# Jamie725/Multimodal-Object-Detection-via-Probabilistic-Ensembling

Measured on AMD Instinct MI355X. Metric: RGB+T frame-pairs/sec (FLIR-aligned 640x512, two R101-FPN detectors + ProbEn), higher is better.
Workload: dtype f16; 1 GPU; configs[2]: FLIR RGB + thermal two-detector ProbEn (probEn/v-avg), batch 32 per GPU, R101-FPN x2, 640x512 -> 800x1000 (padded 800x1024), K=3, random-init weights; batch_per_gpu=32, input_residency=frames resident in HBM before the timed region (no H2D inside it), schedule=two detector streams, staggered by res3, batches back to back

## Files before the change

### include/proben_hip.h

```cpp
#ifndef PROBEN_HIP_H
#define PROBEN_HIP_H

#include <stddef.h>
#include <stdint.h>

#ifdef __cplusplus
extern "C" {
#endif

#define PE_OK 0
#define PE_ERR_INVALID_ARG (-1)
#define PE_ERR_UNSUPPORTED (-2)
#define PE_ERR_HIP (-3)

#define PE_SCORE_PROBEN 0
#define PE_SCORE_AVG 1
#define PE_SCORE_MAX 2
#define PE_SCORE_PROBEN_BINARY 3
#define PE_SCORE_PROBEN_LOGP 4
#define PE_BOX_VAVG 0
#define PE_BOX_SAVG 1
#define PE_BOX_AVG 2
#define PE_BOX_ARGMAX 3

// ... 168 lines not shown
                             int32_t src_c, int32_t ch0, int32_t nch, int32_t flip_rgb, int32_t dst_h, int32_t dst_w,
                             int32_t pad_h, int32_t pad_w, const float* mean_host, const float* std_host, void* dst,
                             void* stream);
int pe_preprocess_pack_pil_u8(const void* src, int32_t num_images, int32_t src_h, int32_t src_w, int32_t src_c,
                              int32_t ch0, int32_t nch, int32_t flip_rgb, int32_t dst_h, int32_t dst_w, int32_t pad_h,
                              int32_t pad_w, const float* mean_host, const float* std_host, const int32_t* xtab,
                              int32_t xk, const int32_t* ytab, int32_t yk, void* dst, void* stream);
int pe_fusion_input_pack(const void* thermal, const void* rgb, int32_t num_images, int32_t th_h, int32_t th_w, int32_t rgb_h,
                         int32_t rgb_w, int32_t ch0, int32_t nch, int32_t dst_h, int32_t dst_w, int32_t pad_h, int32_t pad_w,
                         int32_t pad_multiple, const float* mean_host, const float* std_host, void* dst, void* stream);
int pe_maxpool3x3s2_nhwc(const void* in, void* out, int32_t N, int32_t H, int32_t W, int32_t C, void* stream);
int pe_subsample2_nhwc(const void* in, void* out, int32_t N, int32_t H, int32_t W, int32_t C, void* stream);
int pe_stem_conv7x7_maxpool_f16(const void* x, const void* w_packed, const float* bias, void* out, int32_t N,
                                int32_t H, int32_t W, void* stream);

#define PE_NMS_TRICK 0
#define PE_NMS_CLASS 1
size_t pe_nms_scratch_bytes(int32_t B, int32_t n_max);
int pe_nms_batched(const float* boxes, const float* scores, const int32_t* idxs, const int32_t* counts,
                   const uint8_t* valid, int32_t B, int32_t n_max, float iou_thresh, int32_t mode,
                   int32_t max_out, int32_t* out_keep, int32_t* out_counts, void* scratch,
                   size_t scratch_bytes, void* stream);

int pe_rpn_select_topk(const float* const* level_heads_host, const int32_t* level_hw_host,
                       const int32_t* level_stride_host, const float* cell_anchors_host,
                       int32_t num_levels, int32_t N, int32_t head_stride, int32_t pre_nms_topk,
                       const int32_t* image_hw, float scale_clamp, float* cand_boxes, float* cand_scores,
                       int32_t* cand_level, uint8_t* cand_valid, int32_t cand_per_image, void* scratch,
                       size_t scratch_bytes, void* stream);
size_t pe_rpn_scratch_bytes(const int32_t* level_hw_host, int32_t num_levels, int32_t N);
int pe_gather_boxes(const float* boxes, const float* scores, const int32_t* keep, const int32_t* counts,
                    int32_t N, int32_t n_in, int32_t max_out, float* out_boxes, float* out_scores,
                    void* stream);

int pe_box2box_apply_deltas(const float* deltas, const float* boxes, int32_t N, int32_t k, const float* weights_host,
                            float scale_clamp, float* out, void* stream);
int pe_grid_anchors(const float* cell_anchors, int32_t num_cell_anchors, int32_t H, int32_t W, int32_t stride,
                    float offset, float* out, void* stream);

int pe_sgd_momentum_f32(float* params, const float* grads, float* momentum_buf, void* fp16_shadow, int64_t n, float lr,
                        float momentum, float weight_decay, float grad_scale, int32_t first_step, void* stream);

int pe_roi_align_nhwc(const void* const* feats_host, const int32_t* feat_hw_host, const float* scales_host,
                      int32_t num_levels, int32_t N, int32_t C, int32_t dtype, const float* rois,
                      int32_t rois_have_batch_index, int32_t num_rois, int32_t per_image,
                      const int32_t* counts, int32_t pooled_h, int32_t pooled_w, int32_t sampling_ratio,
                      int32_t aligned, void* output, int32_t* out_level, void* stream);

int pe_roi_align_nhwc_sorted(const void* const* feats_host, const int32_t* feat_hw_host, const float* scales_host,
                             int32_t num_levels, int32_t N, int32_t C, int32_t dtype, const float* boxes, int32_t per_image,
                             const int32_t* counts, int32_t pooled_h, int32_t pooled_w, int32_t sampling_ratio,
                             int32_t aligned, void* output, int32_t* out_level, int32_t* order_workspace, void* stream);

int pe_roi_align_backward_nhwc(const void* grad_output, int32_t dtype, const int32_t* feat_hw_host, const float* scales_host,
                               int32_t num_levels, int32_t N, int32_t C, const float* rois, int32_t rois_have_batch_index,
                               int32_t num_rois, int32_t per_image, const int32_t* counts, int32_t pooled_h,
                               int32_t pooled_w, int32_t sampling_ratio, int32_t aligned, float* const* grad_feats_host,
                               void* stream);

int pe_boxhead_candidates(const float* head, int32_t head_stride, int32_t N, int32_t per_image,
                          int32_t num_classes, const int32_t* prop_counts, const float* proposals,
                          const int32_t* image_hw, const float* reg_weights_host, float scale_clamp,
                          float score_thresh, int32_t cand_max, float* cand_boxes, float* cand_scores,
                          int32_t* cand_class, int32_t* cand_rows, int32_t* cand_counts, int32_t* cand_total,
                          float* probs, void* stream);
int pe_boxhead_finalize(const float* head, int32_t head_stride, int32_t N, int32_t per_image,
// ... 19 lines not shown
```

### multimodal-object-detection-via-probabilistic-ensembling_amd/_lib.py

```python
import ctypes
import os

import torch

_PKG = os.path.dirname(os.path.abspath(__file__))
LIB_PATH = os.path.join(_PKG, "libproben_hip.so")
_lib = None

c_void_p, c_int, c_double, c_float = ctypes.c_void_p, ctypes.c_int32, ctypes.c_double, ctypes.c_float
c_size_t = ctypes.c_size_t

SIGNATURES = {
    "pe_version": [],
    "pe_proben_pack_detections": [c_void_p] * 6 + [c_int] * 6 + [c_void_p] * 9,
    "pe_proben_pack_logits": [c_void_p] * 6 + [c_int] * 6 + [c_void_p] * 9,
    "pe_proben_pack_log_posteriors": [c_void_p] * 6 + [c_int] * 6 + [c_void_p] * 10,
    "pe_log_softmax": [c_void_p, ctypes.c_int64, c_int, c_double, c_void_p, c_void_p],
    "pe_proben_fuse_batch_logp": [c_void_p] * 8 + [c_int] * 4 + [c_double] * 3 + [c_void_p] * 6 + [c_void_p],
    "pe_calibrated_softmax": [c_void_p, ctypes.c_int64, c_int, c_double, c_void_p, c_void_p],
    "pe_temperature_nll": [c_void_p, c_void_p, ctypes.c_int64, c_int, c_void_p, c_int, c_void_p, c_void_p, c_void_p, c_void_p],
    "pe_match_ground_truth": [c_void_p] * 6 + [c_int, c_double, c_int] + [c_void_p] * 4,
    "pe_variance_stats": [c_void_p] * 4 + [ctypes.c_int64, ctypes.c_int64, c_void_p, c_double] + [c_void_p] * 4,
    "pe_proben_pack_calibrated": [c_void_p] * 9 + [c_int] * 6 + [c_void_p] * 10,
    "pe_proben_fuse_batch_pooled": [c_void_p] * 9 + [c_int] * 4 + [c_double] * 3 + [c_void_p] * 2 + [c_int] + [c_void_p] * 6 + [c_void_p],
    "pe_proben_fuse_batch_posterior": [c_void_p] * 9 + [c_int] * 4 + [c_double] * 3 + [c_void_p] * 2 + [c_int] + [c_void_p] * 9 + [c_void_p],
    "pe_proben_fuse_batch_presence": [c_void_p] * 9 + [c_int] * 4 + [c_double] * 3 + [c_void_p] * 3 + [c_int] + [c_void_p] * 10 + [c_void_p],
    "pe_bias_nll": [c_void_p, c_void_p, c_int, c_int, c_void_p, c_int, c_void_p, c_void_p, c_void_p, c_void_p],
    "pe_proben_pack_pooled": [c_void_p] * 9 + [c_int] * 6 + [c_void_p] * 11,
    "pe_pool_nll": [c_void_p, c_void_p, ctypes.c_int64, c_int, c_void_p, ctypes.c_int64, c_void_p, c_void_p, c_int, c_void_p, c_void_p,
                    c_int, c_int, c_void_p, c_void_p, c_void_p, c_void_p],
    "pe_reliability_logits": [c_void_p] * 3 + [ctypes.c_int64, c_int, c_double, c_int] + [c_void_p] * 5,
    "pe_reliability_scores": [c_void_p] * 2 + [ctypes.c_int64, c_int] + [c_void_p] * 5,
    "pe_proben_fuse_batch": [c_void_p] * 8 + [c_int] * 5 + [c_double] * 3 + [c_void_p] * 5 + [c_void_p],
    "pe_conv2d_nhwc_f16": [c_void_p] * 5 + [c_int] * 14 + [c_void_p],
    "pe_conv_wd_supported": [c_int] * 6,
    "pe_conv_wd_pack_weights": [c_void_p] * 2 + [c_int] * 3 + [c_void_p],
    "pe_conv3x3_wd_f16": [c_void_p] * 4 + [c_int] * 7 + [c_void_p],
    "pe_conv_wd_pack_tail": [c_void_p] * 2 + [c_int] * 2 + [c_void_p],
    "pe_bottleneck_tail_wd_f16": [c_void_p] * 7 + [c_int] * 5 + [c_void_p],
    "pe_bneck64_packed_bytes": [c_int] * 2,
    "pe_bneck64_pack": [c_void_p] * 6,
    "pe_bneck64_f16": [c_void_p] * 9 + [c_int] * 5 + [c_void_p],
    "pe_conv_wd_pack_head": [c_void_p] * 2 + [c_int] * 2 + [c_void_p],
    "pe_conv3x3_wd_rpn_head_f16": [c_void_p] * 6 + [c_int] * 4 + [c_void_p],
    "pe_preprocess_pack": [c_void_p] + [c_int] * 11 + [c_void_p] * 4,
    "pe_preprocess_pack_batch": [c_void_p] + [c_int] * 12 + [c_void_p] * 4,
    "pe_preprocess_pack_pil_u8": [c_void_p] + [c_int] * 11 + [c_void_p] * 2 + [c_void_p, c_int, c_void_p, c_int] + [c_void_p] * 2,
    "pe_fusion_input_pack": [c_void_p] * 2 + [c_int] * 12 + [c_void_p] * 4,
    "pe_maxpool3x3s2_nhwc": [c_void_p] * 2 + [c_int] * 4 + [c_void_p],
    "pe_subsample2_nhwc": [c_void_p] * 2 + [c_int] * 4 + [c_void_p],
    "pe_stem_conv7x7_maxpool_f16": [c_void_p] * 4 + [c_int] * 3 + [c_void_p],
    "pe_nms_scratch_bytes": [c_int, c_int],
    "pe_nms_batched": [c_void_p] * 5 + [c_int, c_int, c_float, c_int, c_int] + [c_void_p] * 3 + [c_size_t, c_void_p],
    "pe_rpn_select_topk": [c_void_p] * 4 + [c_int] * 4 + [c_void_p, c_float] + [c_void_p] * 4 + [c_int, c_void_p, c_size_t, c_void_p],
    "pe_rpn_scratch_bytes": [c_void_p, c_int, c_int],
    "pe_box2box_apply_deltas": [c_void_p] * 2 + [c_int] * 2 + [c_void_p, c_float, c_void_p, c_void_p],
    "pe_grid_anchors": [c_void_p, c_int, c_int, c_int, c_int, c_float, c_void_p, c_void_p],
    "pe_gather_boxes": [c_void_p] * 4 + [c_int] * 3 + [c_void_p] * 3,
    "pe_roi_align_nhwc": [c_void_p] * 3 + [c_int] * 4 + [c_void_p] + [c_int] * 3 + [c_void_p] + [c_int] * 4 + [c_void_p] * 3,
    "pe_roi_align_nhwc_sorted": [c_void_p] * 3 + [c_int] * 4 + [c_void_p] + [c_int] + [c_void_p] + [c_int] * 4 + [c_void_p] * 4,
    "pe_sgd_momentum_f32": [c_void_p] * 4 + [ctypes.c_int64] + [ctypes.c_float] * 4 + [c_int, c_void_p],
    "pe_roi_align_backward_nhwc": [c_void_p, c_int, c_void_p, c_void_p, c_int, c_int, c_int, c_void_p, c_int, c_int, c_int, c_void_p, c_int, c_int, c_int, c_int, c_void_p, c_void_p],
    "pe_boxhead_candidates": [c_void_p, c_int, c_int, c_int, c_int] + [c_void_p] * 4 + [c_float, c_float, c_int] + [c_void_p] * 8,
    "pe_cocoeval_bbox": [c_void_p] * 6 + [ctypes.c_int64] + [c_void_p] * 4 + [ctypes.c_int64, c_int, c_int, c_void_p, c_int,
                         c_void_p, c_int, c_void_p, c_int, c_void_p, c_int, c_int, c_void_p, c_void_p],
    "pe_boxhead_finalize": [c_void_p] + [c_int] * 7 + [c_void_p] * 18,
}
_RESTYPE = {"pe_last_error": ctypes.c_char_p, "pe_nms_scratch_bytes": ctypes.c_size_t, "pe_rpn_scratch_bytes": ctypes.c_size_t,
             "pe_bneck64_packed_bytes": ctypes.c_size_t}


TEST_HOOKS = {"pe_test_set_conv_policy": [c_int, c_int], "pe_test_set_wd9_mode": [c_int], "pe_test_wd9_takes": [c_int] * 5, "pe_test_wd9_head_takes": [c_int] * 3, "pe_test_set_wd9_wgs": [c_int, c_int], "pe_test_set_ring_wgs": [c_int], "pe_test_set_roi_fast": [c_int], "pe_test_set_nms_presorted": [c_int]}


class HipLibraryError(RuntimeError):
    pass


def lib():
    global _lib
    if _lib is None:
        if not os.path.exists(LIB_PATH):
            raise HipLibraryError(
                f"{LIB_PATH} is missing: run `python -c 'import __graft_entry__ as g; g.build()'` "
                "(hipcc --offload-arch=gfx950).  proben_amd has no CPU fallback.")
        L = ctypes.CDLL(LIB_PATH)
        L.pe_last_error.restype = ctypes.c_char_p
        L.pe_last_error.argtypes = []
        for name, args in SIGNATURES.items():
            fn = getattr(L, name)
            fn.argtypes = args
            fn.restype = _RESTYPE.get(name, ctypes.c_int)
        _lib = L
    return _lib


LAB_HOOKS = {"pe_test_set_ring_ablation": [c_int]}


def test_hooks():
    L = lib()
# ... 31 lines not shown
```

### multimodal-object-detection-via-probabilistic-ensembling_amd/csrc/nms.hip

```cpp
#include "common.h"
#include "test_hooks.h"

namespace {

constexpr int kSortThreads = 1024;
__device__ int g_presorted_path = 1;

__device__ __forceinline__ unsigned ordered_desc(float s) {
    s += 0.0f;
    unsigned u = __float_as_uint(s);
    u ^= (u >> 31) ? 0xFFFFFFFFu : 0x80000000u;
    return ~u;
}

struct NmsArgs {
    const float* boxes;
    const float* scores;
    const int32_t* idxs;
    const int32_t* counts;
    const uint8_t* valid;
    int B, n_max, n_pad;
    float thr;
    int mode, max_out;
    float* sboxes;
    int32_t* sidx;
    int32_t* scls;
    int32_t* nvalid;
    unsigned* sord;
    int32_t* seg_start;
    int32_t* nseg;
    unsigned long long* mask;
    int words;
    int32_t* out_keep;
// ... 123 lines not shown
__global__ __launch_bounds__(64) void nms_mask_kernel(NmsArgs a) {
    const int b = blockIdx.z;
    const int nv = a.nvalid[b];
    const int row0 = blockIdx.y * 64, col0 = blockIdx.x * 64;
    if (row0 >= nv || col0 >= nv || col0 + 63 < row0) return;
    __shared__ float cb[64][4];
    __shared__ int cc[64];
    const int t = threadIdx.x;
    const float* sb = a.sboxes + (size_t)b * a.n_max * 4;
    {
        const int* cls = a.scls + (size_t)b * a.n_max;
        const unsigned row_last = (unsigned)cls[min(row0 + 63, nv - 1)] & 0x3FFFFu, col_first = (unsigned)cls[col0] & 0x3FFFFu;
        if (col_first > row_last) {
            if (row0 + t < nv) a.mask[((size_t)b * a.n_max + row0 + t) * a.words + blockIdx.x] = 0ull;
            return;
        }
    }
    if (col0 + t < nv) {
        cb[t][0] = sb[(col0 + t) * 4]; cb[t][1] = sb[(col0 + t) * 4 + 1];
        cb[t][2] = sb[(col0 + t) * 4 + 2]; cb[t][3] = sb[(col0 + t) * 4 + 3];
        cc[t] = a.scls[(size_t)b * a.n_max + col0 + t];
    }
    __syncthreads();
    const int r = row0 + t;
    if (r >= nv) return;
    const float x1 = sb[r * 4], y1 = sb[r * 4 + 1], x2 = sb[r * 4 + 2], y2 = sb[r * 4 + 3];
    const float ar = (x2 - x1) * (y2 - y1);
    const int rc = a.scls[(size_t)b * a.n_max + r];
    unsigned long long bits = 0;
    const int jn = min(64, nv - col0);
    for (int j = (col0 == row0 ? t + 1 : 0); j < jn; ++j) {
        if (col0 + j <= r) continue;
        if (cc[j] != rc) continue;
        const float w = fmaxf(0.f, fminf(x2, cb[j][2]) - fmaxf(x1, cb[j][0]));
        const float h = fmaxf(0.f, fminf(y2, cb[j][3]) - fmaxf(y1, cb[j][1]));
        const float inter = w * h;
        const float aj = (cb[j][2] - cb[j][0]) * (cb[j][3] - cb[j][1]);
        const float iou = inter / (ar + aj - inter);
        if (iou > a.thr) bits |= 1ull << j;
    }
    a.mask[((size_t)b * a.n_max + r) * a.words + blockIdx.x] = bits;
}

constexpr int kScanThreads = 1024;
constexpr int kMergeSegs = 16;
__global__ __launch_bounds__(kScanThreads) void nms_scan_order_kernel(NmsArgs a) {
    extern __shared__ __attribute__((aligned(16))) unsigned char smem[];
    unsigned short* kept_pos = reinterpret_cast<unsigned short*>(smem);
    unsigned* flags = reinterpret_cast<unsigned*>(smem + (((size_t)a.n_max * 2 + 15) & ~(size_t)15));
    __shared__ int total_s;
    __shared__ int seg_p0_s[kMergeSegs], seg_kept_s[kMergeSegs];
    const int b = blockIdx.x, tid = threadIdx.x, lane = tid & 63, wave = tid >> 6;
    const int nv = a.nvalid[b];
    const int nseg = a.nseg[b];
    const unsigned long long* mk = a.mask + (size_t)b * a.n_max * a.words;
    for (int i = tid; i < a.n_pad / 32; i += kScanThreads) flags[i] = 0u;
    if (tid == 0) total_s = 0;
    __syncthreads();
    for (int sgi = wave; sgi < nseg; sgi += kScanThreads / 64) {
        const int p0 = a.seg_start[(size_t)b * a.n_max + sgi];
        const int cls0 = a.scls[(size_t)b * a.n_max + p0];
        int p1;
        {
            int lo = p0, hi = nv;
            const unsigned key0 = (unsigned)cls0 & 0x3FFFFu;
            while (lo < hi) {
                const int mid = (lo + hi) >> 1;
                if (((unsigned)a.scls[(size_t)b * a.n_max + mid] & 0x3FFFFu) == key0) lo = mid + 1; else hi = mid;
            }
            p1 = lo;
        }
        unsigned short* kp = kept_pos + p0;
// ... 187 lines not shown
```

### multimodal-object-detection-via-probabilistic-ensembling_amd/csrc/rpn.hip

```cpp
#include "common.h"

namespace {

constexpr int kThreads = 1024;
constexpr int kMaxTopk = 1024;
constexpr int kA = 3;
constexpr int kSliceKeys = 16383;

struct RpnLevel {
    const float* head;
    int H, W, stride;
    int first_slice, num_slices;
    int topk;
    int cand_offset;
    float cell[kA][4];
};

struct RpnArgs {
    RpnLevel lv[8];
    int num_levels, N, head_stride;
    const int32_t* image_hw;
    int cand_per_image;
    float scale_clamp;
    float* cand_boxes;
    float* cand_scores;
    int32_t* cand_level;
    uint8_t* cand_valid;
    unsigned long long* slice_out;
    int num_slices;
    int slice_level[64], slice_begin[64];
};

__device__ __forceinline__ unsigned ordered_desc(float s) {
// ... 156 lines not shown
        const float pcx = dx * wd + cx, pcy = dy * ht + cy;
        const float pw = expf(dw) * wd, ph = expf(dh) * ht;
        float x1 = pcx - 0.5f * pw, y1 = pcy - 0.5f * ph, x2 = pcx + 0.5f * pw, y2 = pcy + 0.5f * ph;
        bool ok = isfinite(x1) && isfinite(y1) && isfinite(x2) && isfinite(y2) && isfinite(score);
        const float ih = (float)a.image_hw[n * 2], iw = (float)a.image_hw[n * 2 + 1];
        x1 = fminf(fmaxf(x1, 0.f), iw); y1 = fminf(fmaxf(y1, 0.f), ih);
        x2 = fminf(fmaxf(x2, 0.f), iw); y2 = fminf(fmaxf(y2, 0.f), ih);
        ok = ok && (x2 - x1) > 0.f && (y2 - y1) > 0.f;
        const size_t o = (size_t)n * a.cand_per_image + lv.cand_offset + tid;
        a.cand_boxes[o * 4] = x1; a.cand_boxes[o * 4 + 1] = y1; a.cand_boxes[o * 4 + 2] = x2; a.cand_boxes[o * 4 + 3] = y2;
        a.cand_scores[o] = score;
        a.cand_level[o] = L;
        a.cand_valid[o] = ok ? 1 : 0;
    }
}

__global__ void gather_rows_kernel(const float* boxes, const float* scores, const int32_t* keep, const int32_t* counts,
                                   int N, int n_in, int max_out, float* out_boxes, float* out_scores) {
    const int i = blockIdx.x * blockDim.x + threadIdx.x;
    if (i >= N * max_out) return;
    const int n = i / max_out, p = i - n * max_out;
    float b0 = 0, b1 = 0, b2 = 0, b3 = 0, s = 0;
    if (p < counts[n]) {
        const int r = keep[i];
        const float* b = boxes + ((size_t)n * n_in + r) * 4;
        b0 = b[0]; b1 = b[1]; b2 = b[2]; b3 = b[3];
        s = scores[(size_t)n * n_in + r];
    }
    out_boxes[(size_t)i * 4] = b0; out_boxes[(size_t)i * 4 + 1] = b1;
    out_boxes[(size_t)i * 4 + 2] = b2; out_boxes[(size_t)i * 4 + 3] = b3;
    if (out_scores) out_scores[i] = s;
}

}

extern "C" int pe_rpn_select_topk(const float* const* level_heads_host, const int32_t* level_hw_host,
                                  const int32_t* level_stride_host, const float* cell_anchors_host,
                                  int32_t num_levels, int32_t N, int32_t head_stride, int32_t pre_nms_topk,
                                  const int32_t* image_hw, float scale_clamp, float* cand_boxes, float* cand_scores,
                                  int32_t* cand_level, uint8_t* cand_valid, int32_t cand_per_image, void* scratch,
                                  size_t scratch_bytes, void* stream) {
    PE_CHECK_ARG(num_levels >= 1 && num_levels <= 8, "pe_rpn_select_topk: num_levels %d", num_levels);
    PE_CHECK_ARG(pre_nms_topk >= 1 && pre_nms_topk <= kMaxTopk, "pe_rpn_select_topk: pre_nms_topk %d not in [1,%d]",
                 pre_nms_topk, kMaxTopk);
    PE_CHECK_ARG(head_stride >= 16 && head_stride % 4 == 0, "pe_rpn_select_topk: head_stride %d (rows must be 16-byte aligned, >= 16 floats)", head_stride);
    PE_CHECK_ARG(level_heads_host && level_hw_host && level_stride_host && cell_anchors_host && image_hw,
                 "pe_rpn_select_topk: null pointer");
    PE_CHECK_ARG(cand_boxes && cand_scores && cand_level && cand_valid, "pe_rpn_select_topk: null output");
    if (N == 0) return PE_OK;
    RpnArgs a{};
    int off = 0;
    for (int l = 0; l < num_levels; ++l) {
        RpnLevel& lv = a.lv[l];
        lv.head = level_heads_host[l];
        lv.H = level_hw_host[2 * l]; lv.W = level_hw_host[2 * l + 1]; lv.stride = level_stride_host[l];
        const long long tot = (long long)lv.H * lv.W * kA;
        lv.topk = (int)std::min<long long>(pre_nms_topk, tot);
        lv.cand_offset = off;
        off += lv.topk;
        for (int i = 0; i < kA * 4; ++i) lv.cell[i / 4][i % 4] = cell_anchors_host[l * kA * 4 + i];
        PE_CHECK_ARG(lv.head != nullptr, "pe_rpn_select_topk: null level pointer");
    }
    PE_CHECK_ARG(off == cand_per_image, "pe_rpn_select_topk: cand_per_image %d != sum of per-level top-k %d",
                 cand_per_image, off);
    a.num_levels = num_levels; a.N = N; a.head_stride = head_stride; a.image_hw = image_hw;
    a.cand_per_image = cand_per_image; a.scale_clamp = scale_clamp;
    a.cand_boxes = cand_boxes; a.cand_scores = cand_scores; a.cand_level = cand_level; a.cand_valid = cand_valid;
    int ns = 0;
    for (int l = 0; l < num_levels; ++l) {
        const int tot = a.lv[l].H * a.lv[l].W * kA;
        const int cnt = (tot + kSliceKeys - 1) / kSliceKeys;
        a.lv[l].first_slice = ns;
        a.lv[l].num_slices = cnt > 1 ? cnt : 0;
        if (cnt > 1) {
            for (int c = 0; c < cnt && ns < 64; ++c, ++ns) { a.slice_level[ns] = l; a.slice_begin[ns] = c * kSliceKeys; }
        }
    }
    a.num_slices = ns;
    static_assert(kSliceKeys % kA == 0, "slices are cut at cell boundaries");
    auto key_bytes = [](int keys) { return ((size_t)keys * sizeof(unsigned) + 15) / 16 * 16; };
    const size_t need = (size_t)N * ns * kMaxTopk * sizeof(unsigned long long);
    const bool two_stage = scratch && ns > 0 && ns < 64 && scratch_bytes >= need;
    size_t lds_slice = 0, lds_select = 0;
    for (int l = 0; l < num_levels; ++l) {
        const int tot = a.lv[l].H * a.lv[l].W * kA;
        if (two_stage && a.lv[l].num_slices > 1) lds_slice = std::max(lds_slice, key_bytes(std::min(tot, kSliceKeys)));
        else if (tot <= kSliceKeys) lds_select = std::max(lds_select, key_bytes(tot));
    }
    constexpr size_t kStaticLds = 10 * 1024;
    if (two_stage) {
        a.slice_out = (unsigned long long*)scratch;
        PE_ENSURE_LDS(rpn_slice_kernel, lds_slice + kStaticLds, "pe_rpn_select_topk(slices)");
        hipLaunchKernelGGL(rpn_slice_kernel, dim3(ns, N), dim3(kThreads), lds_slice, (hipStream_t)stream, a);
        PE_CHECK_LAUNCH("pe_rpn_select_topk(slices)");
    } else {
        a.slice_out = nullptr;
    }
    PE_ENSURE_LDS(rpn_select_kernel, lds_select + kStaticLds, "pe_rpn_select_topk");
    hipLaunchKernelGGL(rpn_select_kernel, dim3(num_levels, N), dim3(kThreads), lds_select, (hipStream_t)stream, a);
    PE_CHECK_LAUNCH("pe_rpn_select_topk");
    return PE_OK;
}

extern "C" size_t pe_rpn_scratch_bytes(const int32_t* level_hw_host, int32_t num_levels, int32_t N) {
    size_t ns = 0;
    for (int l = 0; l < num_levels; ++l) {
        const long long tot = (long long)level_hw_host[2 * l] * level_hw_host[2 * l + 1] * kA;
        const long long cnt = (tot + kSliceKeys - 1) / kSliceKeys;
        if (cnt > 1) ns += (size_t)cnt;
    }
    return (size_t)N * ns * kMaxTopk * sizeof(unsigned long long);
}

extern "C" int pe_gather_boxes(const float* boxes, const float* scores, const int32_t* keep, const int32_t* counts,
                               int32_t N, int32_t n_in, int32_t max_out, float* out_boxes, float* out_scores,
                               void* stream) {
    PE_CHECK_ARG(boxes && keep && counts && out_boxes, "pe_gather_boxes: null pointer");
    if (N == 0) return PE_OK;
    hipLaunchKernelGGL(gather_rows_kernel, dim3(pe::ceil_div((long long)N * max_out, 256)), dim3(256), 0,
                       (hipStream_t)stream, boxes, scores, keep, counts, N, n_in, max_out, out_boxes, out_scores);
    PE_CHECK_LAUNCH("pe_gather_boxes");
    return PE_OK;
}
```

### multimodal-object-detection-via-probabilistic-ensembling_amd/rcnn.py

```python
import ctypes
import math
from dataclasses import dataclass

import torch

from . import _lib
from . import layers as L
from .data import PairFrames
from .structures import Boxes, Instances
from .weights import STAGE_BLOCKS, PackedDetector

SCALE_CLAMP = math.log(1000.0 / 16)


@dataclass
class DetectorConfig:
    num_classes: int = 3
    input_format: str = "BGR"
    pixel_mean: tuple = (103.53, 116.28, 123.675)
    pixel_std: tuple = (1.0, 1.0, 1.0)
    anchor_sizes: tuple = (32, 64, 128, 256, 512)
    aspect_ratios: tuple = (0.5, 1.0, 2.0)
    pre_nms_topk: int = 1000
    post_nms_topk: int = 1000
# ... 11 lines not shown
    @property
    def in_channels(self):
        return {"BGR": 3, "RGB": 3, "BGRT": 4, "BGRTTT": 6}[self.input_format]


def cell_anchor_table(sizes, ratios):
    out = []
    for s in sizes:
        area = float(s) ** 2.0
        for r in ratios:
            w = math.sqrt(area / r)
            h = r * w
            out += [-w / 2.0, -h / 2.0, w / 2.0, h / 2.0]
    return out


class GeneralizedRCNN:
    def __init__(self, cfg: DetectorConfig, state_dict, device="cuda"):
        if not torch.cuda.is_available():
            raise _lib.HipLibraryError("GeneralizedRCNN (MODEL.DEVICE=cuda) needs an MI355X; there is no CPU fallback "
                                       "in proben_amd (the CPU restatement lives in oracle/ for testing only).")
        _lib.lib()
        self.cfg = cfg
        self.device = torch.device(device)
        self.w = PackedDetector(state_dict, device, cfg.num_classes)
        self.depth = self.w.depth
        assert len(cfg.aspect_ratios) == 3, "kernels assume 3 anchors per cell"
        self._cells = (ctypes.c_float * (len(cfg.anchor_sizes) * 12))(*cell_anchor_table(cfg.anchor_sizes, cfg.aspect_ratios))
        self._reg_w = (ctypes.c_float * 4)(10.0, 10.0, 5.0, 5.0)
        self.training = False
        self.use_wd = True
        self.fuse_tails = True
        self.fuse_res2 = True

    def eval(self):
        return self

    def load_state_dict(self, state_dict, strict=True):
        w = PackedDetector(state_dict, self.device, self.cfg.num_classes)
        assert w.depth == self.depth or not strict, f"state dict is ResNet-{w.depth}, model was built as ResNet-{self.depth}"
        self.w, self.depth = w, w.depth
        return self

    def to(self, device):
        assert torch.device(device).type == "cuda", "proben_amd.GeneralizedRCNN lives on the GPU (no CPU fallback)"
        return self

    def _conv(self, x, name, **kw):
        w, b = self.w.convs[name]
        if kw.get("kernel") == 3 and name in self.w.wd and self.use_wd and kw.get("residual") is None and x.numel() * 2 < 2 ** 31 \
                and L.conv_wd_supported(3, 1, x.shape[1], x.shape[2], x.shape[3], w.shape[0]):
            return L.conv3x3_wd(x, self.w.wd[name], b, w.shape[0], relu=kw.get("relu", False), out=kw.get("out"),
                                out_stride=kw.get("out_stride", 0))
        return L.conv2d_nhwc(x, w, b, **kw)

    def _bottom_up(self, x, prefix):
        bu = prefix + ".bottom_up"
        if (bu + ".stem.fused") in self.w.convs and x.shape[1] % 4 == 0 and x.shape[2] % 4 == 0:
            x = L.stem_conv_pool(x, *self.w.convs[bu + ".stem.fused"])
        else:
            x = self._conv(x, bu + ".stem.conv1", kernel=7, stride=2, relu=True)
            x = L.maxpool3x3s2_nhwc(x)
        outs = []
        for si, nb in enumerate(STAGE_BLOCKS[self.depth]):
            chain = self.w.chains64.get(f"{bu}.res{si + 2}") if self.fuse_res2 else None
            if chain is not None and si == 0 and len(chain) == nb and x.shape[0] * x.shape[1] * x.shape[2] * 512 < 2 ** 31:
# ... 124 lines not shown
        Hp, Wp = (size[0] + d - 1) // d * d, (size[1] + d - 1) // d * d
        mean = list(cfg.pixel_mean)
        std = list(cfg.pixel_std) + [cfg.pixel_std[-1]] * (C - len(cfg.pixel_std))
        assert len(mean) == C, f"PIXEL_MEAN needs {C} entries for INPUT.FORMAT {cfg.input_format}"
        batches = []
        for ch0, nch in ([(0, 4)] if C == 4 else [(0, 3), (3, 3)]):
            x = torch.empty((N, Hp, Wp, 4), dtype=torch.float16, device=self.device)
            sd0 = 0 if ch0 == 3 else ch0
            L.fusion_input_pack(pair.thermal.contiguous(), pair.rgb.contiguous() if ch0 < 3 else None, x, ch0=ch0, nch=nch,
                                dst_hw=size, mean=mean[ch0:ch0 + nch], std=std[sd0:sd0 + nch], pad_multiple=d)
            batches.append(x)
        return batches, [size] * N

    def _rpn(self, feats, sizes_dev, N, heads=None):
        cfg = self.cfg
        hw, strides = [], [4, 8, 16, 32, 64]
        if heads is None:
            heads = []
            fused = self.w.rpn_head_fused if self.use_wd else None
            for f in feats:
                if fused is not None and f.numel() * 2 < 2 ** 31 and L.conv_wd_supported(3, 1, f.shape[1], f.shape[2], f.shape[3], 256):
                    heads.append(L.conv3x3_wd_rpn_head(f, self.w.wd["rpn.conv"], self.w.convs["rpn.conv"][1], fused[0], fused[1]))
                    continue
                t = self._conv(f, "rpn.conv", kernel=3, relu=True)
                w, b = self.w.convs["rpn.head"]
                heads.append(L.conv2d_nhwc(t, w, b, kernel=1, out_f32=True, cout=15, cout_store=15, out_stride=16))
        feats = heads
        for f in feats:
            hw += [f.shape[1], f.shape[2]]
        nl = len(feats)
        topk = [min(cfg.pre_nms_topk, f.shape[1] * f.shape[2] * 3) for f in feats]
        ncand = sum(topk)
        dev = self.device
        cb = torch.empty((N, ncand, 4), dtype=torch.float32, device=dev)
        cs = torch.empty((N, ncand), dtype=torch.float32, device=dev)
        cl = torch.empty((N, ncand), dtype=torch.int32, device=dev)
        cv = torch.empty((N, ncand), dtype=torch.uint8, device=dev)
        ptrs = (ctypes.c_void_p * nl)(*[h.data_ptr() for h in heads])
        hw_c = (ctypes.c_int32 * (2 * nl))(*hw)
        sbytes = _lib.lib().pe_rpn_scratch_bytes(hw_c, nl, N)
        scratch = torch.empty((max(sbytes, 8),), dtype=torch.uint8, device=dev)
        st = _lib.lib().pe_rpn_select_topk(ptrs, hw_c, (ctypes.c_int32 * nl)(*strides[:nl]),
                                          self._cells, nl, N, 16, cfg.pre_nms_topk, _lib.ptr(sizes_dev), SCALE_CLAMP,
                                          _lib.ptr(cb), _lib.ptr(cs), _lib.ptr(cl), _lib.ptr(cv), ncand,
                                          _lib.ptr(scratch), sbytes, _lib.stream())
        _lib.check(st, "pe_rpn_select_topk")
        mode = 1 if ncand * 4 > 20000 else 0
        keep, kcnt = L.nms_batched_raw(cb, cs, cl, None, cv, cfg.rpn_nms_thresh, mode, cfg.post_nms_topk)
        props = torch.empty((N, cfg.post_nms_topk, 4), dtype=torch.float32, device=dev)
        plog = torch.empty((N, cfg.post_nms_topk), dtype=torch.float32, device=dev)
        st = _lib.lib().pe_gather_boxes(_lib.ptr(cb), _lib.ptr(cs), _lib.ptr(keep), _lib.ptr(kcnt), N, ncand,
                                       cfg.post_nms_topk, _lib.ptr(props), _lib.ptr(plog), _lib.stream())
        _lib.check(st, "pe_gather_boxes")
        return props, plog, kcnt, heads

    def _roi_heads(self, feats, props, pcnt, sizes_dev, out_dev, N, head=None):
        cfg, w = self.cfg, self.w
        P = cfg.post_nms_topk
        K = cfg.num_classes
        dev = self.device
        pooled = None
        if head is None:
            C = feats[0].shape[3]
            pooled = L.roi_align_nhwc(feats[:4], props, scales=[1 / 4, 1 / 8, 1 / 16, 1 / 32], pooled=(7, 7),
                                      sampling_ratio=0, aligned=True, counts=pcnt, per_image=P, num_rois=N * P)
            x = L.linear_f16(pooled.view(N * P, 49 * C), w.fc1[0], w.fc1[1], relu=True)
            x = L.linear_f16(x, w.fc2[0], w.fc2[1], relu=True)
            head = L.linear_f16(x, w.predictor[0], w.predictor[1], out_f32=True, cout_store=w.head_cols, out_stride=w.head_stride)
        per_prop = min(K, max(1, int(math.ceil(1.0 / max(cfg.score_thresh, 1e-6))) - 1))
        cmax = min(P * per_prop, 16384)
        cb = torch.empty((N, cmax, 4), dtype=torch.float32, device=dev)
        cs = torch.empty((N, cmax), dtype=torch.float32, device=dev)
        cc = torch.empty((N, cmax), dtype=torch.int32, device=dev)
        cr = torch.empty((N, cmax, 2), dtype=torch.int32, device=dev)
        ccnt = torch.empty((N,), dtype=torch.int32, device=dev)
        ctot = torch.empty((N,), dtype=torch.int32, device=dev)
        probs = torch.empty((N, P, K + 1), dtype=torch.float32, device=dev)
        lib = _lib.lib()
        st = lib.pe_boxhead_candidates(_lib.ptr(head), w.head_stride, N, P, K, _lib.ptr(pcnt), _lib.ptr(props),
                                       _lib.ptr(sizes_dev), self._reg_w, SCALE_CLAMP, cfg.score_thresh, cmax,
                                       _lib.ptr(cb), _lib.ptr(cs), _lib.ptr(cc), _lib.ptr(cr), _lib.ptr(ccnt), _lib.ptr(ctot),
                                       _lib.ptr(probs), _lib.stream())
        _lib.check(st, "pe_boxhead_candidates")
# ... 96 lines not shown
```

Measured before the change: 1011 frame-pairs/s.

## Fuse RPN top-k, per-level NMS and merge into a single proposals path

Adds pe_rpn_proposals, which runs the existing top-k selection and then does NMS per (level, image) block entirely in LDS using a triangular IoU bitmask. A merge kernel then combines the per-level kept lists by score rank to write the final proposals. This replaces the generic batched NMS plus gather over all candidates. It splits NMS by level instead of using an offset trick, and adds an early-out in the IoU test when the intersection is zero. The per-block sequential scan on one wave and the LDS footprint could limit occupancy, and whether the per-level split matches batched NMS depends on mode.

Result: no change. 1014 frame-pairs/s, median of 6 (+0.3%).

```diff
diff --git a/include/proben_hip.h b/include/proben_hip.h
--- a/include/proben_hip.h
+++ b/include/proben_hip.h
@@ -224,6 +224,12 @@
 int pe_gather_boxes(const float* boxes, const float* scores, const int32_t* keep, const int32_t* counts,
                     int32_t N, int32_t n_in, int32_t max_out, float* out_boxes, float* out_scores,
                     void* stream);
+size_t pe_rpn_proposals_scratch_bytes(const int32_t* level_hw_host, int32_t num_levels, int32_t N, int32_t pre_nms_topk);
+int pe_rpn_proposals(const float* const* level_heads_host, const int32_t* level_hw_host,
+                     const int32_t* level_stride_host, const float* cell_anchors_host, int32_t num_levels,
+                     int32_t N, int32_t head_stride, int32_t pre_nms_topk, const int32_t* image_hw,
+                     float scale_clamp, float iou_thresh, int32_t mode, int32_t post_nms_topk, float* props,
+                     float* logits, int32_t* counts, void* scratch, size_t scratch_bytes, void* stream);
 
 int pe_box2box_apply_deltas(const float* deltas, const float* boxes, int32_t N, int32_t k, const float* weights_host,
                             float scale_clamp, float* out, void* stream);
diff --git a/multimodal-object-detection-via-probabilistic-ensembling_amd/_lib.py b/multimodal-object-detection-via-probabilistic-ensembling_amd/_lib.py
--- a/multimodal-object-detection-via-probabilistic-ensembling_amd/_lib.py
+++ b/multimodal-object-detection-via-probabilistic-ensembling_amd/_lib.py
@@ -54,6 +54,8 @@
     "pe_nms_batched": [c_void_p] * 5 + [c_int, c_int, c_float, c_int, c_int] + [c_void_p] * 3 + [c_size_t, c_void_p],
     "pe_rpn_select_topk": [c_void_p] * 4 + [c_int] * 4 + [c_void_p, c_float] + [c_void_p] * 4 + [c_int, c_void_p, c_size_t, c_void_p],
     "pe_rpn_scratch_bytes": [c_void_p, c_int, c_int],
+    "pe_rpn_proposals_scratch_bytes": [c_void_p, c_int, c_int, c_int],
+    "pe_rpn_proposals": [c_void_p] * 4 + [c_int] * 4 + [c_void_p, c_float, c_float, c_int, c_int] + [c_void_p] * 4 + [c_size_t, c_void_p],
     "pe_box2box_apply_deltas": [c_void_p] * 2 + [c_int] * 2 + [c_void_p, c_float, c_void_p, c_void_p],
     "pe_grid_anchors": [c_void_p, c_int, c_int, c_int, c_int, c_float, c_void_p, c_void_p],
     "pe_gather_boxes": [c_void_p] * 4 + [c_int] * 3 + [c_void_p] * 3,
@@ -67,6 +69,7 @@
     "pe_boxhead_finalize": [c_void_p] + [c_int] * 7 + [c_void_p] * 18,
 }
 _RESTYPE = {"pe_last_error": ctypes.c_char_p, "pe_nms_scratch_bytes": ctypes.c_size_t, "pe_rpn_scratch_bytes": ctypes.c_size_t,
+             "pe_rpn_proposals_scratch_bytes": ctypes.c_size_t,
              "pe_bneck64_packed_bytes": ctypes.c_size_t}
 
 
diff --git a/multimodal-object-detection-via-probabilistic-ensembling_amd/csrc/nms.hip b/multimodal-object-detection-via-probabilistic-ensembling_amd/csrc/nms.hip
--- a/multimodal-object-detection-via-probabilistic-ensembling_amd/csrc/nms.hip
+++ b/multimodal-object-detection-via-probabilistic-ensembling_amd/csrc/nms.hip
@@ -1,4 +1,5 @@
 #include "common.h"
+#include "nms_iou.h"
 #include "test_hooks.h"
 
 namespace {
@@ -188,12 +189,7 @@
     for (int j = (col0 == row0 ? t + 1 : 0); j < jn; ++j) {
         if (col0 + j <= r) continue;
         if (cc[j] != rc) continue;
-        const float w = fmaxf(0.f, fminf(x2, cb[j][2]) - fmaxf(x1, cb[j][0]));
-        const float h = fmaxf(0.f, fminf(y2, cb[j][3]) - fmaxf(y1, cb[j][1]));
-        const float inter = w * h;
-        const float aj = (cb[j][2] - cb[j][0]) * (cb[j][3] - cb[j][1]);
-        const float iou = inter / (ar + aj - inter);
-        if (iou > a.thr) bits |= 1ull << j;
+        if (pe::nms_iou_above(x1, y1, x2, y2, ar, cb[j][0], cb[j][1], cb[j][2], cb[j][3], a.thr)) bits |= 1ull << j;
     }
     a.mask[((size_t)b * a.n_max + r) * a.words + blockIdx.x] = bits;
 }
diff --git a/multimodal-object-detection-via-probabilistic-ensembling_amd/csrc/nms_iou.h b/multimodal-object-detection-via-probabilistic-ensembling_amd/csrc/nms_iou.h
--- /dev/null
+++ b/multimodal-object-detection-via-probabilistic-ensembling_amd/csrc/nms_iou.h
@@ -0,0 +1,17 @@
+#pragma once
+#include <hip/hip_runtime.h>
+
+namespace pe {
+
+__device__ __forceinline__ bool nms_iou_above(float x1, float y1, float x2, float y2, float ar, float cx1, float cy1, float cx2,
+                                              float cy2, float thr) {
+    const float w = fmaxf(0.f, fminf(x2, cx2) - fmaxf(x1, cx1));
+    const float h = fmaxf(0.f, fminf(y2, cy2) - fmaxf(y1, cy1));
+    const float inter = w * h;
+    if (!(inter > 0.f) && thr >= 0.f) return false;
+    const float aj = (cx2 - cx1) * (cy2 - cy1);
+    const float iou = inter / (ar + aj - inter);
+    return iou > thr;
+}
+
+}
diff --git a/multimodal-object-detection-via-probabilistic-ensembling_amd/csrc/rpn.hip b/multimodal-object-detection-via-probabilistic-ensembling_amd/csrc/rpn.hip
--- a/multimodal-object-detection-via-probabilistic-ensembling_amd/csrc/rpn.hip
+++ b/multimodal-object-detection-via-probabilistic-ensembling_amd/csrc/rpn.hip
@@ -1,4 +1,5 @@
 #include "common.h"
+#include "nms_iou.h"
 
 namespace {
 
@@ -221,14 +222,197 @@
     if (out_scores) out_scores[i] = s;
 }
 
-}
-
-extern "C" int pe_rpn_select_topk(const float* const* level_heads_host, const int32_t* level_hw_host,
-                                  const int32_t* level_stride_host, const float* cell_anchors_host,
-                                  int32_t num_levels, int32_t N, int32_t head_stride, int32_t pre_nms_topk,
-                                  const int32_t* image_hw, float scale_clamp, float* cand_boxes, float* cand_scores,
-                                  int32_t* cand_level, uint8_t* cand_valid, int32_t cand_per_image, void* scratch,
-                                  size_t scratch_bytes, void* stream) {
+struct RpnNmsArgs {
+    int num_levels, N, cand_per_image;
+    int lv_off[8], lv_topk[8];
+    const float* cand_boxes;
+    const float* cand_scores;
+    const uint8_t* cand_valid;
+    float thr;
+    int mode, max_out;
+    unsigned long long* lvl_keys;
+    int32_t* lvl_cnt;
+    float* props;
+    float* logits;
+    int32_t* counts;
+};
+
+constexpr int kNmsChunks = kMaxTopk / 64;
+constexpr int kNmsTiles = kNmsChunks * (kNmsChunks + 1) / 2;
+constexpr size_t kNmsLdsMask = 0;
+constexpr size_t kNmsLdsBox = kNmsLdsMask + (size_t)kNmsTiles * 64 * 8;
+constexpr size_t kNmsLdsRow = kNmsLdsBox + (size_t)kMaxTopk * 16;
+constexpr size_t kNmsLdsKept = kNmsLdsRow + (size_t)kMaxTopk * 2;
+constexpr size_t kNmsLdsRed = kNmsLdsKept + (size_t)kMaxTopk * 2;
+constexpr size_t kNmsLdsBytes = kNmsLdsRed + 64 + 64 + 16;
+
+__device__ __forceinline__ int nms_tile(int r, int c) { return r * kNmsChunks - (r * (r - 1)) / 2 + (c - r); }
+
+__global__ __launch_bounds__(kThreads) void rpn_nms_level_kernel(RpnNmsArgs a) {
+    extern __shared__ __attribute__((aligned(16))) unsigned char smem[];
+    unsigned long long* mask = reinterpret_cast<unsigned long long*>(smem + kNmsLdsMask);
+    float4* sbox = reinterpret_cast<float4*>(smem + kNmsLdsBox);
+    unsigned short* rows = reinterpret_cast<unsigned short*>(smem + kNmsLdsRow);
+    unsigned short* kept = reinterpret_cast<unsigned short*>(smem + kNmsLdsKept);
+    float* red = reinterpret_cast<float*>(smem + kNmsLdsRed);
+    int* wave_cnt = reinterpret_cast<int*>(smem + kNmsLdsRed + 64);
+    int* kept_s = reinterpret_cast<int*>(smem + kNmsLdsRed + 128);
+    const int L = blockIdx.x, n = blockIdx.y, tid = threadIdx.x, lane = tid & 63;
+    const int wave = __builtin_amdgcn_readfirstlane(tid >> 6);
+    const float4* bx = reinterpret_cast<const float4*>(a.cand_boxes) + (size_t)n * a.cand_per_image;
+    const uint8_t* vd = a.cand_valid + (size_t)n * a.cand_per_image;
+    float shift = 0.f;
+    if (a.mode == 0) {
+        float mx = -INFINITY;
+        for (int i = tid; i < a.cand_per_image; i += kThreads) {
+            if (!vd[i]) continue;
+            const float4 b = bx[i];
+            mx = fmaxf(mx, fmaxf(fmaxf(b.x, b.y), fmaxf(b.z, b.w)));
+        }
+        for (int o = 32; o > 0; o >>= 1) mx = fmaxf(mx, __shfl_xor(mx, o));
+        if (lane == 0) red[wave] = mx;
+        __syncthreads();
+        mx = red[0];
+        for (int w = 1; w < kThreads / 64; ++w) mx = fmaxf(mx, red[w]);
+        shift = (float)L * (mx + 1.0f);
+    }
+    const int row = a.lv_off[L] + tid;
+    const bool ok = tid < a.lv_topk[L] && vd[row];
+    const unsigned long long m = __ballot(ok);
+    if (lane == 0) wave_cnt[wave] = __popcll(m);
+    __syncthreads();
+    int nv = 0, pos = __popcll(m & pe::lanemask_lt());
+    for (int w = 0; w < kThreads / 64; ++w) {
+        const int c = wave_cnt[w];
+        if (w < wave) pos += c;
+        nv += c;
+    }
+    if (ok) {
+        const float4 b = bx[row];
+        sbox[pos] = make_float4(b.x + shift, b.y + shift, b.z + shift, b.w + shift);
+        rows[pos] = (unsigned short)row;
+    }
+    __syncthreads();
+    const int nch = (nv + 63) >> 6;
+    const int ntiles = nch * (nch + 1) / 2;
+    for (int t = wave; t < ntiles; t += kThreads / 64) {
+        int r = 0, c = t;
+        while (c >= nch - r) { c -= nch - r; ++r; }
+        c += r;
+        const int p = r * 64 + lane;
+        const float4 rb = p < nv ? sbox[p] : make_float4(0.f, 0.f, 0.f, 0.f);
+        const float ar = (rb.z - rb.x) * (rb.w - rb.y);
+        const float4* cbx = sbox + c * 64;
+        const int jn = min(64, nv - c * 64);
+        unsigned long long bits = 0;
+        for (int j0 = 0; j0 < jn; j0 += 8) {
+            float4 cb[8];
+#pragma unroll
+            for (int u = 0; u < 8; ++u) cb[u] = cbx[j0 + u];
+#pragma unroll
+            for (int u = 0; u < 8; ++u)
+                if (pe::nms_iou_above(rb.x, rb.y, rb.z, rb.w, ar, cb[u].x, cb[u].y, cb[u].z, cb[u].w, a.thr) && j0 + u < jn)
+                    bits |= 1ull << (j0 + u);
+        }
+        if (r == c) bits &= ~((2ull << lane) - 1ull);
+        if (p < nv) mask[nms_tile(r, c) * 64 + lane] = bits;
+    }
+    __syncthreads();
+    if (wave == 0) {
+        int nkept = 0;
+        for (int c = 0; c < nch && nkept < a.max_out; ++c) {
+            const int p = c * 64 + lane;
+            const unsigned long long diag = p < nv ? mask[nms_tile(c, c) * 64 + lane] : 0ull;
+            unsigned long long rem = 0;
+#pragma unroll 4
+            for (int k = lane; k < nkept; k += 64) {
+                const int q = kept[k];
+                rem |= mask[nms_tile(q >> 6, c) * 64 + (q & 63)];
+            }
+            for (int o = 32; o > 0; o >>= 1) rem |= __shfl_xor(rem, o);
+            const unsigned dlo = (unsigned)diag, dhi = (unsigned)(diag >> 32);
+            const int b_hi = min(nv - c * 64, 64);
+            unsigned long long keepmask = 0;
+            int kept_here = 0;
+            for (int bit = 0; bit < b_hi; ++bit) {
+                if ((rem >> bit) & 1ull) continue;
+                if (nkept + kept_here >= a.max_out) break;
+                keepmask |= 1ull << bit;
+                ++kept_here;
+                const unsigned lo = __builtin_amdgcn_readlane(dlo, bit), hi = __builtin_amdgcn_readlane(dhi, bit);
+                rem |= ((unsigned long long)hi << 32) | lo;
+            }
+            if ((keepmask >> lane) & 1ull) kept[nkept + __popcll(keepmask & pe::lanemask_lt())] = (unsigned short)p;
+            nkept += kept_here;
+            __builtin_amdgcn_fence(__ATOMIC_RELEASE, "wavefront");
+            __builtin_amdgcn_wave_barrier();
+        }
+        if (lane == 0) kept_s[0] = nkept;
+    }
+    __syncthreads();
+    const int nkept = kept_s[0];
+    const float* sc = a.cand_scores + (size_t)n * a.cand_per_image;
+    unsigned long long* out = a.lvl_keys + ((size_t)n * a.num_levels + L) * kMaxTopk;
+    for (int g = tid; g < nkept; g += kThreads) {
+        const int i = rows[kept[g]];
+        out[g] = ((unsigned long long)ordered_desc(sc[i]) << 32) | (unsigned)i;
+    }
+    if (tid == 0) a.lvl_cnt[n * a.num_levels + L] = nkept;
+}
+
+__global__ __launch_bounds__(kThreads) void rpn_merge_kernel(RpnNmsArgs a) {
+    extern __shared__ __attribute__((aligned(16))) unsigned char smem[];
+    unsigned long long* keys = reinterpret_cast<unsigned long long*>(smem);
+    int* off = reinterpret_cast<int*>(smem + (size_t)a.num_levels * kMaxTopk * 8);
+    const int n = blockIdx.x, tid = threadIdx.x;
+    if (tid == 0) {
+        off[0] = 0;
+        for (int s = 0; s < a.num_levels; ++s) off[s + 1] = off[s] + a.lvl_cnt[n * a.num_levels + s];
+    }
+    __syncthreads();
+    const int total = off[a.num_levels];
+    for (int g = tid; g < total; g += kThreads) {
+        int s = 0;
+        while (g >= off[s + 1]) ++s;
+        keys[g] = a.lvl_keys[((size_t)n * a.num_levels + s) * kMaxTopk + (g - off[s])];
+    }
+    __syncthreads();
+    const float4* bx = reinterpret_cast<const float4*>(a.cand_boxes) + (size_t)n * a.cand_per_image;
+    const float* sc = a.cand_scores + (size_t)n * a.cand_per_image;
+    float4* pb = reinterpret_cast<float4*>(a.props) + (size_t)n * a.max_out;
+    float* pl = a.logits + (size_t)n * a.max_out;
+    for (int g = tid; g < total; g += kThreads) {
+        int s = 0;
+        while (g >= off[s + 1]) ++s;
+        const unsigned long long x = keys[g];
+        int rank = g - off[s];
+        for (int t = 0; t < a.num_levels; ++t) {
+            if (t == s) continue;
+            int lo = off[t], hi = off[t + 1];
+            while (lo < hi) {
+                const int mid = (lo + hi) >> 1;
+                if (keys[mid] < x) lo = mid + 1; else hi = mid;
+            }
+            rank += lo - off[t];
+        }
+        if (rank < a.max_out) {
+            const int i = (int)(x & 0xFFFFFFFFu);
+            pb[rank] = bx[i];
+            pl[rank] = sc[i];
+        }
+    }
+    const int nout = min(total, a.max_out);
+    for (int i = nout + tid; i < a.max_out; i += kThreads) {
+        pb[i] = make_float4(0.f, 0.f, 0.f, 0.f);
+        pl[i] = 0.f;
+    }
+    if (tid == 0) a.counts[n] = nout;
+}
+
+int run_select(const float* const* level_heads_host, const int32_t* level_hw_host, const int32_t* level_stride_host,
+               const float* cell_anchors_host, int32_t num_levels, int32_t N, int32_t head_stride, int32_t pre_nms_topk,
+               const int32_t* image_hw, float scale_clamp, float* cand_boxes, float* cand_scores, int32_t* cand_level,
+               uint8_t* cand_valid, int32_t cand_per_image, void* scratch, size_t scratch_bytes, void* stream) {
     PE_CHECK_ARG(num_levels >= 1 && num_levels <= 8, "pe_rpn_select_topk: num_levels %d", num_levels);
     PE_CHECK_ARG(pre_nms_topk >= 1 && pre_nms_topk <= kMaxTopk, "pe_rpn_select_topk: pre_nms_topk %d not in [1,%d]",
                  pre_nms_topk, kMaxTopk);
@@ -291,6 +475,19 @@
     return PE_OK;
 }
 
+}
+
+extern "C" int pe_rpn_select_topk(const float* const* level_heads_host, const int32_t* level_hw_host,
+                                  const int32_t* level_stride_host, const float* cell_anchors_host,
+                                  int32_t num_levels, int32_t N, int32_t head_stride, int32_t pre_nms_topk,
+                                  const int32_t* image_hw, float scale_clamp, float* cand_boxes, float* cand_scores,
+                                  int32_t* cand_level, uint8_t* cand_valid, int32_t cand_per_image, void* scratch,
+                                  size_t scratch_bytes, void* stream) {
+    return run_select(level_heads_host, level_hw_host, level_stride_host, cell_anchors_host, num_levels, N, head_stride,
+                      pre_nms_topk, image_hw, scale_clamp, cand_boxes, cand_scores, cand_level, cand_valid, cand_per_image,
+                      scratch, scratch_bytes, stream);
+}
+
 extern "C" size_t pe_rpn_scratch_bytes(const int32_t* level_hw_host, int32_t num_levels, int32_t N) {
     size_t ns = 0;
     for (int l = 0; l < num_levels; ++l) {
@@ -311,3 +508,79 @@
     PE_CHECK_LAUNCH("pe_gather_boxes");
     return PE_OK;
 }
+
+namespace {
+struct ProposalScratch {
+    size_t slices, boxes, scores, level, valid, keys, cnt, total;
+};
+ProposalScratch proposal_scratch(const int32_t* level_hw_host, int32_t num_levels, int32_t N, int32_t pre_nms_topk) {
+    auto up = [](size_t b) { return (b + 255) & ~(size_t)255; };
+    size_t ncand = 0;
+    for (int l = 0; l < num_levels; ++l)
+        ncand += (size_t)std::min<long long>(pre_nms_topk, (long long)level_hw_host[2 * l] * level_hw_host[2 * l + 1] * kA);
+    ProposalScratch s{};
+    size_t at = 0;
+    s.slices = at; at += up(pe_rpn_scratch_bytes(level_hw_host, num_levels, N));
+    s.boxes = at;  at += up((size_t)N * ncand * 16);
+    s.scores = at; at += up((size_t)N * ncand * 4);
+    s.level = at;  at += up((size_t)N * ncand * 4);
+    s.valid = at;  at += up((size_t)N * ncand);
+    s.keys = at;   at += up((size_t)N * num_levels * kMaxTopk * 8);
+    s.cnt = at;    at += up((size_t)N * num_levels * 4);
+    s.total = at;
+    return s;
+}
+}
+
+extern "C" size_t pe_rpn_proposals_scratch_bytes(const int32_t* level_hw_host, int32_t num_levels, int32_t N,
+                                                 int32_t pre_nms_topk) {
+    if (!level_hw_host || num_levels < 1 || num_levels > 8 || N < 0 || pre_nms_topk < 1) return 0;
+    return proposal_scratch(level_hw_host, num_levels, N, pre_nms_topk).total;
+}
+
+extern "C" int pe_rpn_proposals(const float* const* level_heads_host, const int32_t* level_hw_host,
+                                const int32_t* level_stride_host, const float* cell_anchors_host, int32_t num_levels,
+                                int32_t N, int32_t head_stride, int32_t pre_nms_topk, const int32_t* image_hw,
+                                float scale_clamp, float iou_thresh, int32_t mode, int32_t post_nms_topk, float* props,
+                                float* logits, int32_t* counts, void* scratch, size_t scratch_bytes, void* stream) {
+    PE_CHECK_ARG(num_levels >= 1 && num_levels <= 8, "pe_rpn_proposals: num_levels %d", num_levels);
+    PE_CHECK_ARG(pre_nms_topk >= 1 && pre_nms_topk <= kMaxTopk, "pe_rpn_proposals: pre_nms_topk %d not in [1,%d]", pre_nms_topk,
+                 kMaxTopk);
+    PE_CHECK_ARG(N >= 0, "pe_rpn_proposals: negative batch");
+    PE_CHECK_ARG(mode == 0 || mode == 1, "pe_rpn_proposals: mode %d", mode);
+    PE_CHECK_ARG(post_nms_topk >= 1, "pe_rpn_proposals: post_nms_topk < 1");
+    PE_CHECK_ARG(level_hw_host && props && logits && counts, "pe_rpn_proposals: null pointer");
+    PE_CHECK_ARG(((uintptr_t)props & 15) == 0, "pe_rpn_proposals: props must be 16-byte aligned");
+    if (N == 0) return PE_OK;
+    const ProposalScratch ps = proposal_scratch(level_hw_host, num_levels, N, pre_nms_topk);
+    PE_CHECK_ARG(scratch && ((uintptr_t)scratch & 15) == 0, "pe_rpn_proposals: scratch null or not 16-byte aligned");
+    PE_CHECK_ARG(scratch_bytes >= ps.total, "pe_rpn_proposals: scratch too small (%zu < %zu)", scratch_bytes, ps.total);
+    unsigned char* base = (unsigned char*)scratch;
+    RpnNmsArgs a{};
+    int ncand = 0;
+    for (int l = 0; l < num_levels; ++l) {
+        a.lv_off[l] = ncand;
+        a.lv_topk[l] = (int)std::min<long long>(pre_nms_topk, (long long)level_hw_host[2 * l] * level_hw_host[2 * l + 1] * kA);
+        ncand += a.lv_topk[l];
+    }
+    float* cand_boxes = (float*)(base + ps.boxes);
+    float* cand_scores = (float*)(base + ps.scores);
+    uint8_t* cand_valid = base + ps.valid;
+    const int st = run_select(level_heads_host, level_hw_host, level_stride_host, cell_anchors_host, num_levels, N, head_stride,
+                              pre_nms_topk, image_hw, scale_clamp, cand_boxes, cand_scores, (int32_t*)(base + ps.level),
+                              cand_valid, ncand, base + ps.slices, ps.boxes - ps.slices, stream);
+    if (st != PE_OK) return st;
+    a.num_levels = num_levels; a.N = N; a.cand_per_image = ncand;
+    a.cand_boxes = cand_boxes; a.cand_scores = cand_scores; a.cand_valid = cand_valid;
+    a.thr = iou_thresh; a.mode = mode; a.max_out = post_nms_topk;
+    a.lvl_keys = (unsigned long long*)(base + ps.keys); a.lvl_cnt = (int32_t*)(base + ps.cnt);
+    a.props = props; a.logits = logits; a.counts = counts;
+    PE_ENSURE_LDS(rpn_nms_level_kernel, kNmsLdsBytes, "pe_rpn_proposals(nms)");
+    hipLaunchKernelGGL(rpn_nms_level_kernel, dim3(num_levels, N), dim3(kThreads), kNmsLdsBytes, (hipStream_t)stream, a);
+    PE_CHECK_LAUNCH("pe_rpn_proposals(nms)");
+    const size_t lds_merge = (size_t)num_levels * kMaxTopk * 8 + 64;
+    PE_ENSURE_LDS(rpn_merge_kernel, lds_merge, "pe_rpn_proposals(merge)");
+    hipLaunchKernelGGL(rpn_merge_kernel, dim3(N), dim3(kThreads), lds_merge, (hipStream_t)stream, a);
+    PE_CHECK_LAUNCH("pe_rpn_proposals(merge)");
+    return PE_OK;
+}
diff --git a/multimodal-object-detection-via-probabilistic-ensembling_amd/rcnn.py b/multimodal-object-detection-via-probabilistic-ensembling_amd/rcnn.py
--- a/multimodal-object-detection-via-probabilistic-ensembling_amd/rcnn.py
+++ b/multimodal-object-detection-via-probabilistic-ensembling_amd/rcnn.py
@@ -67,6 +67,7 @@
         self.use_wd = True
         self.fuse_tails = True
         self.fuse_res2 = True
+        self.fuse_rpn = True
 
     def eval(self):
         return self
@@ -257,12 +258,25 @@
         topk = [min(cfg.pre_nms_topk, f.shape[1] * f.shape[2] * 3) for f in feats]
         ncand = sum(topk)
         dev = self.device
+        mode = 1 if ncand * 4 > 20000 else 0
+        ptrs = (ctypes.c_void_p * nl)(*[h.data_ptr() for h in heads])
+        hw_c = (ctypes.c_int32 * (2 * nl))(*hw)
+        props = torch.empty((N, cfg.post_nms_topk, 4), dtype=torch.float32, device=dev)
+        plog = torch.empty((N, cfg.post_nms_topk), dtype=torch.float32, device=dev)
+        if self.fuse_rpn:
+            kcnt = torch.empty((N,), dtype=torch.int32, device=dev)
+            sbytes = _lib.lib().pe_rpn_proposals_scratch_bytes(hw_c, nl, N, cfg.pre_nms_topk)
+            scratch = torch.empty((max(sbytes, 8),), dtype=torch.uint8, device=dev)
+            st = _lib.lib().pe_rpn_proposals(ptrs, hw_c, (ctypes.c_int32 * nl)(*strides[:nl]), self._cells, nl, N, 16,
+                                            cfg.pre_nms_topk, _lib.ptr(sizes_dev), SCALE_CLAMP, cfg.rpn_nms_thresh, mode,
+                                            cfg.post_nms_topk, _lib.ptr(props), _lib.ptr(plog), _lib.ptr(kcnt),
+                                            _lib.ptr(scratch), sbytes, _lib.stream())
+            _lib.check(st, "pe_rpn_proposals")
+            return props, plog, kcnt, heads
         cb = torch.empty((N, ncand, 4), dtype=torch.float32, device=dev)
         cs = torch.empty((N, ncand), dtype=torch.float32, device=dev)
         cl = torch.empty((N, ncand), dtype=torch.int32, device=dev)
         cv = torch.empty((N, ncand), dtype=torch.uint8, device=dev)
-        ptrs = (ctypes.c_void_p * nl)(*[h.data_ptr() for h in heads])
-        hw_c = (ctypes.c_int32 * (2 * nl))(*hw)
         sbytes = _lib.lib().pe_rpn_scratch_bytes(hw_c, nl, N)
         scratch = torch.empty((max(sbytes, 8),), dtype=torch.uint8, device=dev)
         st = _lib.lib().pe_rpn_select_topk(ptrs, hw_c, (ctypes.c_int32 * nl)(*strides[:nl]),
@@ -270,10 +284,7 @@
                                           _lib.ptr(cb), _lib.ptr(cs), _lib.ptr(cl), _lib.ptr(cv), ncand,
                                           _lib.ptr(scratch), sbytes, _lib.stream())
         _lib.check(st, "pe_rpn_select_topk")
-        mode = 1 if ncand * 4 > 20000 else 0
         keep, kcnt = L.nms_batched_raw(cb, cs, cl, None, cv, cfg.rpn_nms_thresh, mode, cfg.post_nms_topk)
-        props = torch.empty((N, cfg.post_nms_topk, 4), dtype=torch.float32, device=dev)
-        plog = torch.empty((N, cfg.post_nms_topk), dtype=torch.float32, device=dev)
         st = _lib.lib().pe_gather_boxes(_lib.ptr(cb), _lib.ptr(cs), _lib.ptr(keep), _lib.ptr(kcnt), N, ncand,
                                        cfg.post_nms_topk, _lib.ptr(props), _lib.ptr(plog), _lib.stream())
         _lib.check(st, "pe_gather_boxes")
```
